# genetics-statistics/GEMMA

Hardware: AMD Instinct MI355X
Metric: SNPs/s (-lmm 1 Wald) at n=20k on 1/2/4/8 MI355X; U^T x HBM GB/s vs roofline (higher is better)
Workload: dtype f64 (U^T x as int8-digit MFMA products with exact int32 accumulation; every column of U scaled by its exact maximum and rounded to 6 base-256 digits = 2^-48 of that maximum -- fp64 keeps 2^-53 per entry; value_strict / strict_leg (7g6m: U^T x at or below the fp64 GEMM's own error) and fp64_gemm_path

## Files before the change

gemma_amd/_lib.py:

```python
import ctypes as C
import os

HERE = os.path.dirname(os.path.abspath(__file__))
LIB_PATH = os.path.join(HERE, "libgemma_hip.so")

SYMBOLS = [
    "gemma_hip_init", "gemma_hip_shutdown", "gemma_hip_abi_version", "gemma_hip_strerror",
    "gemma_hip_last_error", "gemma_hip_device_info", "gemma_hip_dgemm", "gemma_hip_dgemm_d",
    "gemma_hip_kin_begin", "gemma_hip_kin_add", "gemma_hip_kin_add_d", "gemma_hip_kin_end",
    "gemma_hip_kin_end_d", "gemma_hip_kin_loco_d", "gemma_hip_snp_qc", "gemma_hip_center", "gemma_hip_center_d", "gemma_hip_eigh",
    "gemma_hip_eigh_d", "gemma_hip_eigh_reserve", "gemma_hip_eigh_release", "gemma_hip_dbg_eigh_last", "gemma_hip_eigh_sharded_d", "gemma_hip_eigh_kept_K_sharded", "gemma_hip_calc_utx", "gemma_hip_lmm_setup", "gemma_hip_lmm_setup_d",
    "gemma_hip_lmm_null", "gemma_hip_lmm_set_indicator", "gemma_hip_lmm_batch", "gemma_hip_lmm_batch_d",
    "gemma_hip_lmm_assoc_d", "gemma_hip_lmm_finish", "gemma_hip_lm_setup", "gemma_hip_lm_batch", "gemma_hip_lm_batch_d",
    "gemma_hip_lm_finish", "gemma_hip_profile_enable",
    "gemma_hip_profile_read", "gemma_hip_dbg_tridiag", "gemma_hip_dbg_stedc", "gemma_hip_dbg_eigh2", "gemma_hip_dbg_utx", "gemma_hip_lmm_gene_batch", "gemma_hip_lmm_gene_batch_d", "gemma_hip_lmm_set_env",
    "gemma_hip_lmm_gxe_batch", "gemma_hip_lmm_gxe_batch_d",
    "gemma_hip_mvlmm_null", "gemma_hip_mvlmm_set", "gemma_hip_mvlmm_batch", "gemma_hip_mvlmm_batch_d",
    "gemma_hip_kin_end_keep", "gemma_hip_kept_K_get", "gemma_hip_eigh_kept_K", "gemma_hip_eigh_keep", "gemma_hip_kept_n",
    "gemma_hip_kept_bcast", "gemma_hip_kept_U_get", "gemma_hip_calc_utx_kept", "gemma_hip_lmm_setup_kept", "gemma_hip_kept_release",
    "gemma_hip_comm_unique_id", "gemma_hip_comm_init", "gemma_hip_comm_info", "gemma_hip_comm_bcast_d",
    "gemma_hip_comm_allreduce_sum_d", "gemma_hip_comm_finalize", "gemma_hip_comm_selftest", "gemma_hip_comm_stats", "gemma_hip_dbg_i8_digits", "gemma_hip_dbg_last_utx_path", "gemma_hip_lmm_batch_submit", "gemma_hip_lmm_batch_collect",
    "gemma_hip_dbg_last_utx_kernel", "gemma_hip_dbg_last_block_missing", "gemma_hip_dbg_last_i8_post", "gemma_hip_reload_env", "gemma_hip_lmm_batch_pipe_d", "gemma_hip_lmm_pipe_flush",
    "gemma_hip_spd_inverse", "gemma_hip_spd_inverse_d", "gemma_hip_vc_setup", "gemma_hip_vc_setup_d", "gemma_hip_vc_he",
    "gemma_hip_vc_reml", "gemma_hip_vc_timing", "gemma_hip_vc_release",
    "gemma_hip_ridge_setup", "gemma_hip_ridge_setup_d", "gemma_hip_ridge_setup_kept", "gemma_hip_ridge_set_r",
    "gemma_hip_ridge_set_indicator", "gemma_hip_ridge_batch", "gemma_hip_ridge_batch_d", "gemma_hip_ridge_finish",
    "gemma_hip_prdt_begin", "gemma_hip_prdt_add", "gemma_hip_prdt_add_d", "gemma_hip_prdt_add_bv", "gemma_hip_prdt_add_bv_d",
    "gemma_hip_prdt_end", "gemma_hip_prdt_kin", "gemma_hip_prdt_kin_mv_apply", "gemma_hip_prdt_kin_mv_apply_d", "gemma_hip_prdt_kin_mv",
    "gemma_hip_mqs_begin", "gemma_hip_mqs_add", "gemma_hip_mqs_add_d", "gemma_hip_mqs_end", "gemma_hip_mqs_get",
    "gemma_hip_mqs_S", "gemma_hip_mqs_S_d", "gemma_hip_mqs_release",
    "gemma_hip_cor_begin", "gemma_hip_cor_block", "gemma_hip_cor_block_d", "gemma_hip_cor_release",
    "gemma_hip_ci_begin", "gemma_hip_ci_xwz", "gemma_hip_ci_xwz_d", "gemma_hip_ci_xwz_end", "gemma_hip_ci_xtxwz",
    "gemma_hip_ci_xtxwz_d", "gemma_hip_ci_release",
    "gemma_hip_lmm_multi_setup", "gemma_hip_lmm_multi_setup_d", "gemma_hip_lmm_multi_setup_kept", "gemma_hip_lmm_multi_batch",
    "gemma_hip_lmm_multi_batch_d",
    "gemma_hip_lmm_score_panel_setup", "gemma_hip_lmm_score_panel_setup_d", "gemma_hip_lmm_score_panel_setup_kept",
    "gemma_hip_lmm_score_panel_batch", "gemma_hip_lmm_score_panel_batch_d", "gemma_hip_lmm_score_panel_assoc_d",
# ... 156 lines not shown
    L.gemma_hip_lmm_multi_batch_d.argtypes = [ci, vp, sz, sz, vp, vp]
    L.gemma_hip_lmm_score_panel_setup.argtypes = [C.POINTER(LmmCfg), sz, dp, dp, dp, dp, dp]
    L.gemma_hip_lmm_score_panel_setup_d.argtypes = [C.POINTER(LmmCfg), sz, dp, dp, dp, dp, dp, vp]
    L.gemma_hip_lmm_score_panel_setup_kept.argtypes = [C.POINTER(LmmCfg), sz, dp, dp, dp]
    L.gemma_hip_lmm_score_panel_batch.argtypes = [ci, vp, sz, sz, vp]
    L.gemma_hip_lmm_score_panel_batch_d.argtypes = [ci, vp, sz, sz, vp, vp]
    L.gemma_hip_lmm_score_panel_assoc_d.argtypes = [dp, sz, sz, vp, vp]
    L.gemma_hip_lmm_score_panel_hits_batch.argtypes = [ci, vp, sz, sz, C.c_double, vp, sz, vp, vp]
    L.gemma_hip_lmm_score_panel_hits_batch_d.argtypes = [ci, vp, sz, sz, C.c_double, vp, sz, vp, vp, vp]
    L.gemma_hip_lmm_score_panel_hits_assoc_d.argtypes = [dp, sz, sz, C.c_double, vp, sz, vp, vp, vp]
    L.gemma_hip_lmm_null_panel.argtypes = [sz, sz, sz, dp, dp, dp, cd, cd, sz, cd, vp, dp, dp]
    L.gemma_hip_lmm_null_panel_d.argtypes = [sz, sz, sz, dp, dp, dp, cd, cd, sz, cd, vp, dp, dp, vp]
    L.gemma_hip_dbg_i8_digits.argtypes = [sz, C.POINTER(ci)]
    L.gemma_hip_dbg_last_utx_path.argtypes = [C.POINTER(ci)]
    L.gemma_hip_dbg_last_utx_kernel.argtypes = [C.POINTER(UtxKernelInfo)]
    L.gemma_hip_dbg_last_block_missing.argtypes = [C.POINTER(ci)]
    L.gemma_hip_dbg_last_i8_post.argtypes = [C.POINTER(C.c_long), C.POINTER(C.c_long), C.POINTER(ci)]
    L.gemma_hip_reload_env.argtypes = []
    L.gemma_hip_lmm_batch_pipe_d.argtypes = [ci, vp, sz, sz, vp, vp]
    L.gemma_hip_lmm_pipe_flush.argtypes = [vp]
    L.gemma_hip_lmm_batch_submit.argtypes = [ci, vp, sz, sz]
    L.gemma_hip_lmm_batch_collect.argtypes = [vp, C.POINTER(sz)]
    L.gemma_hip_comm_unique_id.argtypes = [vp]
    L.gemma_hip_comm_init.argtypes = [vp, ci, ci]
    L.gemma_hip_comm_info.argtypes = [C.POINTER(ci), C.POINTER(ci), C.POINTER(ci)]
    L.gemma_hip_comm_bcast_d.argtypes = [vp, sz, ci, vp]
    L.gemma_hip_comm_allreduce_sum_d.argtypes = [dp, sz, vp]
    L.gemma_hip_comm_selftest.argtypes = [vp]
    L.gemma_hip_comm_stats.argtypes = [C.POINTER(CommStats)]
    L.gemma_hip_spd_inverse.argtypes = [dp, sz, sz, C.POINTER(cd), C.POINTER(C.c_long)]
# ... 56 lines not shown
```

gemma_amd/api.py:

```python
import collections
import ctypes as C

import numpy as np

from . import _lib as L

SUMSTAT_DTYPE = np.dtype([(k, "f8") for k in
                          ("beta", "se", "lambda_remle", "lambda_mle", "p_wald", "p_lrt", "p_score",
                           "logl_H1")])
SCORE_DTYPE = np.dtype([(k, "f8") for k in ("beta", "se", "p_score")])
SCORE_HIT_DTYPE = np.dtype([("snp", "u4"), ("pheno", "u4"), ("beta", "f8"), ("se", "f8"), ("p_score", "f8")])
SCORE_BEST_DTYPE = np.dtype([("beta", "f8"), ("se", "f8"), ("p_score", "f8"), ("snp", "i8")])
NULL_DTYPE = np.dtype([(k, "f8") for k in ("l_mle_null", "logl_mle_H0", "l_remle_null", "logl_remle_H0", "pve", "pve_se", "vg_remle",
                                             "ve_remle")])
LMM_BATCH_SIZE = 20000
K_BATCH_SIZE = 20000


def _is_torch(x):
    return type(x).__module__.startswith("torch")


def _np64(a, name):
    if not isinstance(a, np.ndarray) or a.dtype != np.float64:
# ... 77 lines not shown
    L.check(L.lib().gemma_hip_dbg_last_utx_path(C.byref(p)), "dbg_last_utx_path")
    return p.value


def last_utx_kernel():
    k = L.UtxKernelInfo()
    L.check(L.lib().gemma_hip_dbg_last_utx_kernel(C.byref(k)), "dbg_last_utx_kernel")
    return {"variant": k.variant, "rows": k.rows, "digits": k.digits, "fuse": k.fuse, "raster": k.raster,
            "launches": k.launches, "name": k.name.decode()}


def last_block_missing():
    a = C.c_int()
    L.check(L.lib().gemma_hip_dbg_last_block_missing(C.byref(a)), "dbg_last_block_missing")
    return a.value


def reload_env():
    L.check(L.lib().gemma_hip_reload_env(), "reload_env")


def fast_dgemm(TransA, TransB, alpha, A, B, beta, Cm):
    ta, tb = TransA.upper()[0], TransB.upper()[0]
    M, N = Cm.shape
    if ta not in "NT" or tb not in "NT":
        raise L.GemmaHipError(L.EINVAL, "fast_dgemm", "bad transpose flag")
    Ka = A.shape[0] if ta == "T" else A.shape[1]
    Ma = A.shape[1] if ta == "T" else A.shape[0]
    Kb = B.shape[1] if tb == "T" else B.shape[0]
    Nb = B.shape[0] if tb == "T" else B.shape[1]
# ... 1871 lines not shown
```

gemma_amd/csrc/abi_kept_comm.inc.h:

```cpp

extern "C" int gemma_hip_kin_end_keep(size_t *ns_used, int allreduce) {
  NEED_INIT();
  if (!g_ctx.kin_active) return fail(GEMMA_HIP_ESTATE, "kin_end before kin_begin");
  const size_t n = g_ctx.kin_n;
  size_t ns = g_ctx.kin_ns;
  {
    int rc = kin_fold_i8(nullptr);
    if (rc) return rc;
  }
  if (allreduce && g_ctx.comm.active && g_ctx.comm.world > 1) {
    std::string err;
    if (g_ctx.comm.allreduce_sum(g_ctx.kin_K.as<double>(), n * n, nullptr, err)) return fail(GEMMA_HIP_ERUNTIME, "%s", err.c_str());
    if (g_ctx.scratch.reserve(16)) return fail(GEMMA_HIP_ENOMEM, "kin_end_keep: scratch");
    double cnt = (double)ns;
    HIPCHK(hipMemcpy(g_ctx.scratch.p, &cnt, 8, hipMemcpyHostToDevice));
    if (g_ctx.comm.allreduce_sum(g_ctx.scratch.as<double>(), 1, nullptr, err)) return fail(GEMMA_HIP_ERUNTIME, "%s", err.c_str());
    HIPCHK(hipMemcpy(&cnt, g_ctx.scratch.p, 8, hipMemcpyDeviceToHost));
    ns = (size_t)(cnt + 0.5);
  }
  if (ns_used) *ns_used = ns;
  const double scale = ns ? 1.0 / (double)ns : 1.0;
  const unsigned nb = (unsigned)((n + 31) / 32);
  hipLaunchKernelGGL(symm_fill_scale_kernel, dim3(nb, nb), dim3(32, 8), 0, 0, g_ctx.kin_K.as<double>(), (long)n, (long)n,
                     scale);
// ... 309 lines not shown
  out->bcast_pieces = st.bcast_pieces;
  out->allreduce_bytes = st.allreduce_bytes;
  out->bcast_bytes = st.bcast_bytes;
  out->allreduce_s = st.allreduce_s;
  out->bcast_s = st.bcast_s;
  return GEMMA_HIP_OK;
}


extern "C" int gemma_hip_dbg_last_utx_kernel(gemma_utx_kernel_info *info) {
  if (!info) return fail(GEMMA_HIP_EINVAL, "dbg_last_utx_kernel: null");
  *info = g_ctx.last_utx_kernel;
  return GEMMA_HIP_OK;
}

extern "C" int gemma_hip_dbg_last_block_missing(int *any) {
  NEED_INIT();
  if (!any) return fail(GEMMA_HIP_EINVAL, "dbg_last_block_missing: null");
  *any = -1;
  if (g_ctx.i8_flag_at < 0 || !g_ctx.i8_rowsur.p) return GEMMA_HIP_OK;
  HIPCHK(hipDeviceSynchronize());
  HIPCHK(hipMemcpy(any, g_ctx.i8_rowsur.as<int>() + g_ctx.i8_flag_at, sizeof(int), hipMemcpyDeviceToHost));
  return GEMMA_HIP_OK;
}

extern "C" int gemma_hip_dbg_last_i8_post(long *short_rows, long *long_rows, int *epilogue) {
  NEED_INIT();
  if (!short_rows || !long_rows || !epilogue) return fail(GEMMA_HIP_EINVAL, "dbg_last_i8_post: null");
  *short_rows = *long_rows = -1;
  *epilogue = g_ctx.i8_last_epi;
// ... 30 lines not shown
```

gemma_amd/csrc/abi_lmm_stage.inc.h:

```cpp

static void slot_swap(Ctx::PhenoSlot &p) {
  std::swap(g_ctx.assoc_proto, p.proto);
  std::swap(g_ctx.Uty, p.Uty);
  std::swap(g_ctx.grid_R, p.grid_R); std::swap(g_ctx.grid_F, p.grid_F);
  std::swap(g_ctx.cheb_R, p.cheb_R); std::swap(g_ctx.cheb_F, p.cheb_F);
  std::swap(g_ctx.carry, p.carry);
  std::swap(g_ctx.carry_flip, p.carry_flip);
  std::swap(g_ctx.grid_geom, p.grid_geom); std::swap(g_ctx.cheb_geom, p.cheb_geom);
  std::swap(g_ctx.cheb_mid, p.cheb_mid); std::swap(g_ctx.cheb_inv_half, p.cheb_inv_half);
  std::swap(g_ctx.cheb_qmask, p.cheb_qmask);
}
static void multi_release() {
  for (auto &p : g_ctx.slots) {
    p.grid_R.release(); p.grid_F.release(); p.cheb_R.release(); p.cheb_F.release(); p.carry.release();
  }
  g_ctx.slots.clear();
  g_ctx.multi_Yt.release(); g_ctx.multi_R.release(); g_ctx.multi_T_buf.release();
  g_ctx.multi_T = 0;
  g_ctx.multi_G = 0;
}
static void score_release() {
  g_ctx.score_R.release(); g_ctx.score_Pyy.release(); g_ctx.score_Yt.release(); g_ctx.score_lam.release(); g_ctx.score_bad.release();
  g_ctx.score_fthr.release(); g_ctx.score_cells.release(); g_ctx.score_hits.release(); g_ctx.score_cnt.release(); g_ctx.score_best.release();
  g_ctx.score_fthr_p = -1.0;
// ... 228 lines not shown
  hipLaunchKernelGGL(grid_weights_kernel, dim3((unsigned)((r_elems + 255) / 256)), dim3(256), 0, s, k, gg, (int)c,
                     g_ctx.grid_R.as<double>());
  HIPCHK(hipGetLastError());
  hipLaunchKernelGGL(grid_fixed_kernel, dim3((unsigned)gg.nq), dim3(256), 0, s, k, (int)c, g_ctx.grid_F.as<double>());
  HIPCHK(hipGetLastError());
  g_ctx.grid_geom = gg;
  a.grid_F = g_ctx.grid_F.as<double>();
  a.grid_ld = (int)(nb * 16);
  a.grid_nq = gg.nq;
  a.grid_xa0 = gg.nbx * 16;
  a.have_grid = 1;
  return make_cheb(s);
}

static bool table_v2_enabled() { return g_ctx.knobs.table_v2 != 0; }
static int table_ksplit(int nc) { return std::max(1, std::min(16, nc / 32)); }
template <int NBX, int NBA, int RG>
static int launch_table_v2_t(const GridGeom &gg, const double *UtX, size_t l, size_t ld, const double *R, double *T,
                             const TableGather *tg, int nint, hipStream_t s) {
  constexpr int NB16 = (NBX + NBA) * 16;
  const size_t rows_per_block = (size_t)RG * 16 * 4;
  const size_t bx = (l + rows_per_block - 1) / rows_per_block;
  const int ksplit = table_ksplit(gg.nc);
  const size_t planes = tg ? (size_t)nint : 1;
  if (g_ctx.table_P.reserve(planes * (size_t)ksplit * l * NB16 * 8))
    return fail(GEMMA_HIP_ENOMEM, "lmm_assoc: table partial sums (%zu bytes)", planes * (size_t)ksplit * l * NB16 * 8);
  TableV2 a;
  a.UtX = UtX; a.ld = (long)ld; a.l = (long)l; a.n = (int)g_ctx.cfg.n; a.nc = gg.nc; a.ksplit = ksplit; a.Rp = R;
  a.P = g_ctx.table_P.as<double>(); a.cap = (long)l;
  if (tg) a.tg = *tg; else a.tg = TableGather();
  const long total = (long)l * NB16;
// ... 2 lines not shown
    if (pf) hipLaunchKernelGGL((table_v2_kernel<NBX, NBA, RG, true, true>), dim3((unsigned)bx, (unsigned)ksplit, (unsigned)nint), dim3(256), 0, s, a);
    else hipLaunchKernelGGL((table_v2_kernel<NBX, NBA, RG, true, false>), dim3((unsigned)bx, (unsigned)ksplit, (unsigned)nint), dim3(256), 0, s, a);
    HIPCHK(hipGetLastError());
    hipLaunchKernelGGL(table_reduce_kernel<true>, dim3((unsigned)((total + 255) / 256), (unsigned)nint), dim3(256), 0, s,
                       a.P, ksplit, a.cap, NB16, (long)l, tg->count, T);
  } else {
    if (pf) hipLaunchKernelGGL((table_v2_kernel<NBX, NBA, RG, false, true>), dim3((unsigned)bx, (unsigned)ksplit), dim3(256), 0, s, a);
    else hipLaunchKernelGGL((table_v2_kernel<NBX, NBA, RG, false, false>), dim3((unsigned)bx, (unsigned)ksplit), dim3(256), 0, s, a);
    HIPCHK(hipGetLastError());
    hipLaunchKernelGGL(table_reduce_kernel<false>, dim3((unsigned)((total + 255) / 256)), dim3(256), 0, s, a.P, ksplit,
                       a.cap, NB16, (long)l, (const int *)nullptr, T);
  }
  HIPCHK(hipGetLastError());
  return GEMMA_HIP_OK;
}
static int launch_table_v2(const GridGeom &gg, const double *UtX, size_t l, size_t ld, const double *R, double *T,
                           const TableGather *tg, int nint, hipStream_t s) {
  switch (gg.nba) {
  case 3: return launch_table_v2_t<2, 3, 4>(gg, UtX, l, ld, R, T, tg, nint, s);
  case 5: return launch_table_v2_t<2, 5, 2>(gg, UtX, l, ld, R, T, tg, nint, s);
  case 6: return launch_table_v2_t<2, 6, 2>(gg, UtX, l, ld, R, T, tg, nint, s);
  case 8: return launch_table_v2_t<2, 8, 2>(gg, UtX, l, ld, R, T, tg, nint, s);
  default: return fail(GEMMA_HIP_ERUNTIME, "lmm_assoc: no table kernel for %d column blocks", gg.nba);
  }
}

static int launch_grid_table(const double *UtX, size_t l, size_t ld, hipStream_t s) {
  const GridGeom &gg = g_ctx.grid_geom;
  const size_t nb = (size_t)(gg.nbx + gg.nba);
  if (g_ctx.grid_T.reserve(l * nb * 16 * 8)) return fail(GEMMA_HIP_ENOMEM, "lmm_assoc: fixed-lambda table");
  const unsigned grid = (unsigned)((l + 15) / 16);
  const double *R = g_ctx.grid_R.as<double>();
// ... 288 lines not shown
```

gemma_amd/csrc/gemma_hip.hip:

```cpp
#include <hip/hip_runtime.h>

#include <cmath>
#include <cstdarg>
#include <cstdio>
#include <cstdlib>
#include <cstring>
#include <string>
#include <vector>

#include "../../include/gemma_hip.h"
#include "tu_common.h"
#include "dgemm.h"
#include "eigh_tu.h"
#include "vc_tu.h"
#include "prdt_tu.h"
#include "mqs_tu.h"
#include "cor_tu.h"
#include "ingest.h"
#include "lm_assoc.h"
#include "lmm_assoc.h"
#include "lmm_grid.h"
#include "lmm_score_panel.h"
#include "lmm_null_panel.h"
#include "i8gemm.h"
#include "i8gemm_sparse.h"
#include "i8gemm_sparse2.h"
#include "i8gemm_sparse2_r16.h"
#include "plink_records.h"
#include "i8gemm_dense16.h"
#include "qc.h"
#include "mvlmm.hip.h"
#include "comm.hip.h"
#include "kin_i8.h"
#include "i8_plan.h"

using namespace gemma_hip;

namespace {

struct StageProf {
  std::vector<std::pair<hipEvent_t, hipEvent_t>> ev;
  double acc_ms = 0.0;
  long launches = 0;
};

struct Knobs {
  I8Switches i8;
  int i8_digits = 0;
  int i8_scale_max = 1;
  int dosage_i8 = 1;
  int dosage_rows = 16;
  int table_v2 = 1;
  int table_pf = 0;
  int multi_table = 1;
  int force_generic = 0;
  int assoc_variant = 44;
  int mvlmm_rt = 0;
  int pipe_cus = 64;
  int kin_i8 = 1, kin_upper = 1, kin_lists = 1, kin_lists_oom = 0;
  long long kin_list_cap = 0;
  static int geti(const char *name, int dflt) {
    const char *e = getenv(name);
    return (e && *e) ? atoi(e) : dflt;
  }
  void load() {
    i8.utx_i8 = geti("GEMMA_HIP_UTX_I8", 1);
    const int dg = geti("GEMMA_HIP_I8_DIGITS", 0);
    i8_digits = (dg == 6 || dg == 7) ? dg : 0;
// ... 14 lines not shown
    const char *eep = getenv("GEMMA_HIP_I8_EPILOGUE");
    i8.epilogue = (eep && eep[0] == '0') ? 0 : 1;
    i8.epi_depth = geti("GEMMA_HIP_I8_EPI_DEPTH", 4) <= 1 ? 1 : 4;
    const char *edr = getenv("GEMMA_HIP_I8_DIRECT");
    i8.direct = (edr && edr[0] == '0') ? 0 : 1;
    const char *ed = getenv("GEMMA_HIP_UTX_DOSAGE_I8");
    dosage_i8 = (ed && ed[0] == '0') ? 0 : 1;
    dosage_rows = geti("GEMMA_HIP_DOSAGE_ROWS", 16) == 32 ? 32 : 16;
    const char *eo = getenv("GEMMA_HIP_OVERLAP");
    i8.overlap = (eo && eo[0] == '1') ? 1 : 0;
    i8.chunks = geti("GEMMA_HIP_OVERLAP_CHUNKS", 4);
    const char *et = getenv("GEMMA_HIP_TABLE_V2");
    table_v2 = (et && et[0] == '0') ? 0 : 1;
    const char *ep = getenv("GEMMA_HIP_TABLE_PF");
    table_pf = (ep && ep[0] == '1') ? 1 : 0;
    const char *em = getenv("GEMMA_HIP_MULTI_TABLE");
    multi_table = (em && em[0] == '0') ? 0 : 1;
    const char *eg = getenv("GEMMA_HIP_FORCE_GENERIC");
    force_generic = (eg && eg[0] == '1') ? 1 : 0;
    assoc_variant = geti("GEMMA_HIP_ASSOC_VARIANT", 44);
    const char *er = getenv("GEMMA_HIP_MVLMM_RT");
    mvlmm_rt = (er && er[0] == '1') ? 1 : 0;
    pipe_cus = geti("GEMMA_HIP_PIPE_CUS", 64);
    const char *k1 = getenv("GEMMA_HIP_KIN_I8"), *k2 = getenv("GEMMA_HIP_KIN_UPPER"), *k3 = getenv("GEMMA_HIP_KIN_LISTS");
    const char *k4 = getenv("GEMMA_HIP_KIN_LISTS_OOM"), *k5 = getenv("GEMMA_HIP_KIN_LIST_CAP");
    kin_i8 = (k1 && k1[0] == '0') ? 0 : 1;
    kin_upper = (k2 && k2[0] == '0') ? 0 : 1;
    kin_lists = (k3 && k3[0] == '0') ? 0 : 1;
    kin_lists_oom = (k4 && k4[0] == '1') ? 1 : 0;
    kin_list_cap = (k5 && *k5) ? atoll(k5) : 0;
// ... 41 lines not shown
  } xp;
  int kin_tmap_tm = 0, kin_tmap_tn = 0, kin_tmap_count = 0;

  bool lmm_active = false;
  gemma_lmm_cfg cfg;
  const double *U = nullptr, *eval = nullptr, *Uty = nullptr;
  DevBuf own_U, own_eval, own_Uty, own_UtW, UtWt, idx_map;
  size_t ni_total = 0;
  bool have_map = false;
  DevBuf X, UtX, stage_in, stage_out, carry;
  DevBuf grid_R, grid_F, grid_T;
  DevBuf cheb_R, cheb_F, cheb_T, cheb_slots, cheb_list, cheb_count, cheb_D, cheb_Ck, cheb_Gk, cheb_Lk, cheb_iv, cheb_dends, cheb_res;
  double cheb_mid[ASSOC_MAX_REGION], cheb_inv_half[ASSOC_MAX_REGION];
  GridGeom cheb_geom;
  DevBuf table_P;
  DevBuf gxe_env, gxe_UtWt, gxe_Z, gxe_UtZ, gxe_flip;
  bool gxe_ready = false;
  double gxe_lnbeta = 0.0;
  DevBuf mv_Yt, mv_out;
  DevBuf mv_scratch;
  bool mv_ready = false, mv_gxe = false;
  size_t mv_d = 0;
  MvArgs mv_proto;
  DevBuf i8_Bt, i8_q, i8_qinv, i8_cmax, i8_A, i8_C, i8_mean;
  unsigned long long cheb_qmask = 0;
  struct RasterSlot {
    DevBuf dev;
    std::vector<int2> host;
    int tm = 0, tn = 0, rb = 0, xcds = 8;
    unsigned long long used = 0;
// ... 331 lines not shown
```

gemma_amd/csrc/lmm_grid.h:

```cpp
#pragma once
#include <hip/hip_runtime.h>
#include "dgemm.h"
#include "lmm_assoc.h"

namespace gemma_hip {

constexpr int GRID_FIX_LD = 16;

struct GridGeom {
  int nq;
  int nbx;
  int nba;
  int nc;
};

__global__ void grid_weights_kernel(AssocArgs g, GridGeom gg, int c, double *__restrict__ Rp);

__global__ __launch_bounds__(256) void grid_fixed_kernel(AssocArgs g, int c, double *__restrict__ F);

struct TableGather {
  const int *list;
  const int *count;
  long cap;
  long rp_stride;
// ... 2 lines not shown
template <int NBX, int NBA, bool GATHER>
__global__ __launch_bounds__(256) void grid_table_kernel(const double *__restrict__ UtX, long ld, long l, int n,
                                                        int nc, const double *__restrict__ Rp,
                                                        double *__restrict__ T, TableGather tg);

struct TableV2 {
  const double *UtX;
  long ld;
  long l;
  int n, nc;
  int ksplit;
  const double *Rp;
  double *P;
  long cap;
  TableGather tg;
};

template <int NBX, int NBA, int RG, bool GATHER, bool PF>
__global__ __launch_bounds__(256, PF ? 1 : 2) void table_v2_kernel(TableV2 a);

template <bool GATHER>
__global__ __launch_bounds__(256) void table_reduce_kernel(const double *__restrict__ P, int ksplit, long cap, int nb16,
                                                          long l, const int *__restrict__ count, double *__restrict__ T);

constexpr int MULTI_NBA = 8, MULTI_RG = 2, MULTI_GMAX = 4;
struct MultiWeights {
  const double *Uty[MULTI_GMAX];
  int G;
};

__global__ void grid_weights_multi_kernel(AssocArgs g, GridGeom gg, int c, MultiWeights mw, double *__restrict__ Rp);
struct TableMulti {
  const double *P;
  int ksplit;
// ... 61 lines not shown
  T void table_v2_kernel<2, 3, 4, false, true>(TableV2); \
  T void table_v2_kernel<2, 3, 4, true, false>(TableV2); \
  T void table_v2_kernel<2, 3, 4, true, true>(TableV2); \
  T void table_v2_kernel<2, 5, 2, false, false>(TableV2); \
  T void table_v2_kernel<2, 5, 2, false, true>(TableV2); \
  T void table_v2_kernel<2, 5, 2, true, false>(TableV2); \
  T void table_v2_kernel<2, 5, 2, true, true>(TableV2); \
  T void table_v2_kernel<2, 6, 2, false, false>(TableV2); \
  T void table_v2_kernel<2, 6, 2, false, true>(TableV2); \
  T void table_v2_kernel<2, 6, 2, true, false>(TableV2); \
  T void table_v2_kernel<2, 6, 2, true, true>(TableV2); \
  T void table_v2_kernel<2, 8, 2, false, false>(TableV2); \
  T void table_v2_kernel<2, 8, 2, false, true>(TableV2); \
  T void table_v2_kernel<2, 8, 2, true, false>(TableV2); \
  T void table_v2_kernel<2, 8, 2, true, true>(TableV2); \
  T void table_reduce_kernel<false>(const double *, int, long, int, long, const int *, double *); \
  T void table_reduce_kernel<true>(const double *, int, long, int, long, const int *, double *); \
  T void cheb_scan_kernel<1>(AssocArgs, ChebScanArgs); \
  T void cheb_scan_kernel<2>(AssocArgs, ChebScanArgs); \
  T void cheb_scan_kernel<3>(AssocArgs, ChebScanArgs); \
  T void cheb_scan_kernel<4>(AssocArgs, ChebScanArgs); \
  T void cheb_search_kernel<1>(AssocArgs, ChebSearchArgs); \
  T void cheb_search_kernel<2>(AssocArgs, ChebSearchArgs); \
  T void cheb_search_kernel<3>(AssocArgs, ChebSearchArgs); \
  T void cheb_search_kernel<4>(AssocArgs, ChebSearchArgs);
#ifndef GEMMA_HIP_KERNEL_BODIES
LMM_GRID_INSTANCES(extern template __global__)
#endif

}
// ... 1 lines not shown
```

gemma_amd/csrc/lmm_grid.hip.h:

```cpp
#pragma once
#include <hip/hip_runtime.h>
#include "dgemm.h"
#include "lmm_assoc.hip.h"
#define GEMMA_HIP_KERNEL_BODIES
#include "lmm_grid.h"

namespace gemma_hip {

__device__ __forceinline__ double grid_weight(const double *__restrict__ eval, const double *lam_grid, int q, long k) {
  if (q == 0) return 1.0;
  const int gi = (q - 1) >> 1;
  const double h = recip(eval[k] * lam_grid[gi] + 1.0);
  return ((q - 1) & 1) ? h * h : h;
}

__global__ void grid_weights_kernel(AssocArgs g, GridGeom gg, int c, double *__restrict__ Rp) {
  const long total = (long)gg.nc * (gg.nbx + gg.nba) * 256;
  const long e = (long)blockIdx.x * blockDim.x + threadIdx.x;
  if (e >= total) return;
  const int j = (int)(e & 3), col = (int)((e >> 2) & 15), kq = (int)((e >> 6) & 3);
  const long r = e >> 8;
  const int nb = gg.nbx + gg.nba;
  const int cb = (int)(r % nb);
  const long chunk = r / nb;
// ... 221 lines not shown
    TV2_MFMA(rbA, xvA);
  }
#undef TV2_LOAD
#undef TV2_MFMA
  double *P = a.P + ((long)(kint * a.ksplit + ks) * a.cap) * (NB * 16);
#pragma unroll
  for (int g = 0; g < RG; ++g)
#pragma unroll
    for (int b = 0; b < NB; ++b)
#pragma unroll
      for (int r = 0; r < 4; ++r) {
        const long srow = s0 + g * 16 + kq + 4 * r;
        if (srow < l) P[srow * (NB * 16) + b * 16 + i] = acc[g][b][r];
      }
}
template <bool GATHER>
__global__ __launch_bounds__(256) void table_reduce_kernel(const double *__restrict__ P, int ksplit, long cap, int nb16,
                                                          long l, const int *__restrict__ count, double *__restrict__ T) {
  const int kint = GATHER ? blockIdx.y : 0;
  if (GATHER) l = count[kint];
  const long e = (long)blockIdx.x * 256 + threadIdx.x;
  if (e >= l * nb16) return;
  const long row = e / nb16;
  const int col = (int)(e - row * nb16);
  const double *p = P + ((long)kint * ksplit * cap + row) * nb16 + col;
  double v = 0.0;
  for (int ks = 0; ks < ksplit; ++ks) v += p[(long)ks * cap * nb16];
  if (GATHER)
    T[((long)kint * nb16 + col) * cap + row] = v;
  else
// ... 231 lines not shown
```

include/gemma_hip.h:

```cpp
#ifndef GEMMA_HIP_H
#define GEMMA_HIP_H

#include <stddef.h>
#include <stdint.h>

#ifdef __cplusplus
extern "C" {
#endif

#define GEMMA_HIP_ABI_VERSION 4

enum {
  GEMMA_HIP_OK = 0,
  GEMMA_HIP_EINVAL = 1,
  GEMMA_HIP_ENODEV = 2,
  GEMMA_HIP_ENOMEM = 3,
  GEMMA_HIP_ERUNTIME = 4,
  GEMMA_HIP_ESTATE = 5,
  GEMMA_HIP_ENOCONV = 6,
  GEMMA_HIP_ENOTPD = 7
};

typedef struct {
  double beta, se, lambda_remle, lambda_mle, p_wald, p_lrt, p_score, logl_H1;
// ... 206 lines not shown
  GEMMA_UTX_KERNEL_RECORDS_R16 = 4,
  GEMMA_UTX_KERNEL_DOSAGE_I8 = 5,
  GEMMA_UTX_KERNEL_DOSAGE_I8_R16 = 6,
  GEMMA_UTX_KERNEL_COUNT = 7
};
typedef struct {
  int variant;
  int rows;
  int digits;
  int fuse;
  int raster;
  long launches;
  char name[64];
} gemma_utx_kernel_info;
int gemma_hip_dbg_last_utx_kernel(gemma_utx_kernel_info *info);
int gemma_hip_dbg_last_block_missing(int *any);
int gemma_hip_dbg_last_i8_post(long *short_rows, long *long_rows, int *epilogue);
int gemma_hip_reload_env(void);
int gemma_hip_dbg_i8_digits(size_t n, int *digits);

int gemma_hip_spd_inverse(double *A, size_t n, size_t lda, double *logdet, long *bad_pivot);
int gemma_hip_spd_inverse_d(double *A_d, size_t n, size_t lda, double *logdet, long *bad_pivot, void *stream);

int gemma_hip_vc_setup(size_t n, size_t n_vc, const double *const *K, size_t ldk, const double *W, size_t n_cvt, const double *y);
int gemma_hip_vc_setup_d(size_t n, size_t n_vc, const double *const *K_d, size_t ldk, const double *W, size_t n_cvt,
                         const double *y);
int gemma_hip_vc_he(double *sigma2, double *se_sigma2, double *pve, double *se_pve, double *pve_total, double *se_pve_total);
int gemma_hip_vc_reml(int noconstrain, double *sigma2, double *se_sigma2, double *pve, double *se_pve, double *pve_total,
                      double *se_pve_total, int *iterations, int *status, long *counts, double *iter_sigma2, size_t iter_cap);
int gemma_hip_vc_timing(double *t5);
// ... 61 lines not shown
```

Baseline: 364,700.

## Add double-buffered LDS table kernel with occupancy-aware row-group planning

Adds a table_v3 kernel that stages the R coefficients through double-buffered shared memory and prefetches the next chunk of R and UtX into registers while the current MFMA stage computes. A new planner picks the row-group count per workgroup so the last round of work items fills most CU slots, and caps the grid for the gathered case using a grid-stride loop. The default table form is set to 3, so dense (non-gather) table builds take the new path, while gather builds keep the old v2 kernel unless form 4 is requested. This adds LDS pressure and extra index arithmetic in exchange for hiding global-load latency and reducing tail imbalance.

```diff
diff --git a/gemma_amd/_lib.py b/gemma_amd/_lib.py
--- a/gemma_amd/_lib.py
+++ b/gemma_amd/_lib.py
@@ -20,7 +20,7 @@
     "gemma_hip_kept_bcast", "gemma_hip_kept_U_get", "gemma_hip_calc_utx_kept", "gemma_hip_lmm_setup_kept", "gemma_hip_kept_release",
     "gemma_hip_comm_unique_id", "gemma_hip_comm_init", "gemma_hip_comm_info", "gemma_hip_comm_bcast_d",
     "gemma_hip_comm_allreduce_sum_d", "gemma_hip_comm_finalize", "gemma_hip_comm_selftest", "gemma_hip_comm_stats", "gemma_hip_dbg_i8_digits", "gemma_hip_dbg_last_utx_path", "gemma_hip_lmm_batch_submit", "gemma_hip_lmm_batch_collect",
-    "gemma_hip_dbg_last_utx_kernel", "gemma_hip_dbg_last_block_missing", "gemma_hip_dbg_last_i8_post", "gemma_hip_reload_env", "gemma_hip_lmm_batch_pipe_d", "gemma_hip_lmm_pipe_flush",
+    "gemma_hip_dbg_last_utx_kernel", "gemma_hip_dbg_last_table", "gemma_hip_dbg_last_block_missing", "gemma_hip_dbg_last_i8_post", "gemma_hip_reload_env", "gemma_hip_lmm_batch_pipe_d", "gemma_hip_lmm_pipe_flush",
     "gemma_hip_spd_inverse", "gemma_hip_spd_inverse_d", "gemma_hip_vc_setup", "gemma_hip_vc_setup_d", "gemma_hip_vc_he",
     "gemma_hip_vc_reml", "gemma_hip_vc_timing", "gemma_hip_vc_release",
     "gemma_hip_ridge_setup", "gemma_hip_ridge_setup_d", "gemma_hip_ridge_setup_kept", "gemma_hip_ridge_set_r",
@@ -207,6 +207,7 @@
     L.gemma_hip_dbg_i8_digits.argtypes = [sz, C.POINTER(ci)]
     L.gemma_hip_dbg_last_utx_path.argtypes = [C.POINTER(ci)]
     L.gemma_hip_dbg_last_utx_kernel.argtypes = [C.POINTER(UtxKernelInfo)]
+    L.gemma_hip_dbg_last_table.argtypes = [C.POINTER(ci), C.POINTER(ci), C.POINTER(ci), C.POINTER(C.c_long)]
     L.gemma_hip_dbg_last_block_missing.argtypes = [C.POINTER(ci)]
     L.gemma_hip_dbg_last_i8_post.argtypes = [C.POINTER(C.c_long), C.POINTER(C.c_long), C.POINTER(ci)]
     L.gemma_hip_reload_env.argtypes = []
diff --git a/gemma_amd/api.py b/gemma_amd/api.py
--- a/gemma_amd/api.py
+++ b/gemma_amd/api.py
@@ -115,6 +115,12 @@
     a = C.c_int()
     L.check(L.lib().gemma_hip_dbg_last_block_missing(C.byref(a)), "dbg_last_block_missing")
     return a.value
+
+
+def last_table():
+    f, d, g, n = C.c_int(), C.c_int(), C.c_int(), C.c_long()
+    L.check(L.lib().gemma_hip_dbg_last_table(C.byref(f), C.byref(d), C.byref(g), C.byref(n)), "dbg_last_table")
+    return {"form": f.value, "rg_dense": d.value, "rg_gather": g.value, "launches": n.value}
 
 
 def reload_env():
diff --git a/gemma_amd/csrc/abi_kept_comm.inc.h b/gemma_amd/csrc/abi_kept_comm.inc.h
--- a/gemma_amd/csrc/abi_kept_comm.inc.h
+++ b/gemma_amd/csrc/abi_kept_comm.inc.h
@@ -347,6 +347,14 @@
   return GEMMA_HIP_OK;
 }
 
+extern "C" int gemma_hip_dbg_last_table(int *form, int *rg_dense, int *rg_gather, long *launches) {
+  if (launches) *launches = g_ctx.table_launches;
+  if (form) *form = g_ctx.last_table_form;
+  if (rg_dense) *rg_dense = g_ctx.last_table_rg[0];
+  if (rg_gather) *rg_gather = g_ctx.last_table_rg[1];
+  return GEMMA_HIP_OK;
+}
+
 extern "C" int gemma_hip_dbg_last_block_missing(int *any) {
   NEED_INIT();
   if (!any) return fail(GEMMA_HIP_EINVAL, "dbg_last_block_missing: null");
diff --git a/gemma_amd/csrc/abi_lmm_stage.inc.h b/gemma_amd/csrc/abi_lmm_stage.inc.h
--- a/gemma_amd/csrc/abi_lmm_stage.inc.h
+++ b/gemma_amd/csrc/abi_lmm_stage.inc.h
@@ -266,7 +266,6 @@
 }
 
 static bool table_v2_enabled() { return g_ctx.knobs.table_v2 != 0; }
-static int table_ksplit(int nc) { return std::max(1, std::min(16, nc / 32)); }
 template <int NBX, int NBA, int RG>
 static int launch_table_v2_t(const GridGeom &gg, const double *UtX, size_t l, size_t ld, const double *R, double *T,
                              const TableGather *tg, int nint, hipStream_t s) {
@@ -299,8 +298,65 @@
   HIPCHK(hipGetLastError());
   return GEMMA_HIP_OK;
 }
+template <int NBX, int NBA, int RG, bool GATHER>
+static void launch_table_v3_rg(const TablePlan &p, const TableV2 &a, hipStream_t s) {
+  hipLaunchKernelGGL((table_v3_kernel<NBX, NBA, RG, GATHER>), dim3(p.grid), dim3(256), 0, s, a);
+}
+template <int NBX, int NBA, bool GATHER>
+static int launch_table_v3_g(const TablePlan &p, const TableV2 &a, hipStream_t s) {
+  constexpr int NB = NBX + NBA;
+  switch (p.rg) {
+  case 1: launch_table_v3_rg<NBX, NBA, 1, GATHER>(p, a, s); break;
+  case 2:
+    if constexpr (NB <= 7) {
+      launch_table_v3_rg<NBX, NBA, 2, GATHER>(p, a, s);
+      break;
+    }
+  default: return fail(GEMMA_HIP_ERUNTIME, "lmm_assoc: no table kernel for %d row groups at %d column blocks", p.rg, NB);
+  }
+  return GEMMA_HIP_OK;
+}
+template <int NBX, int NBA>
+static int launch_table_v3_t(const GridGeom &gg, const double *UtX, size_t l, size_t ld, const double *R, double *T,
+                             const TableGather *tg, int nint, hipStream_t s) {
+  constexpr int NB16 = (NBX + NBA) * 16;
+  if (l == 0) return GEMMA_HIP_OK;
+  const TablePlan p = table_plan((long)l, gg.nc, g_ctx.prop.multiProcessorCount, NBX + NBA, tg ? nint : 0);
+  const size_t planes = tg ? (size_t)nint : 1;
+  if (g_ctx.table_P.reserve(planes * (size_t)p.ksplit * l * NB16 * 8))
+    return fail(GEMMA_HIP_ENOMEM, "lmm_assoc: table partial sums (%zu bytes)", planes * (size_t)p.ksplit * l * NB16 * 8);
+  TableV2 a;
+  a.UtX = UtX; a.ld = (long)ld; a.l = (long)l; a.n = (int)g_ctx.cfg.n; a.nc = gg.nc; a.ksplit = p.ksplit; a.Rp = R;
+  a.P = g_ctx.table_P.as<double>(); a.cap = (long)l; a.nint = tg ? nint : 0;
+  if (tg) a.tg = *tg; else a.tg = TableGather();
+  const long total = (long)l * NB16;
+  int rc = tg ? launch_table_v3_g<NBX, NBA, true>(p, a, s) : launch_table_v3_g<NBX, NBA, false>(p, a, s);
+  if (rc) return rc;
+  HIPCHK(hipGetLastError());
+  if (tg)
+    hipLaunchKernelGGL(table_reduce_kernel<true>, dim3((unsigned)((total + 255) / 256), (unsigned)nint), dim3(256), 0, s,
+                       a.P, p.ksplit, a.cap, NB16, (long)l, tg->count, T);
+  else
+    hipLaunchKernelGGL(table_reduce_kernel<false>, dim3((unsigned)((total + 255) / 256)), dim3(256), 0, s, a.P, p.ksplit,
+                       a.cap, NB16, (long)l, (const int *)nullptr, T);
+  HIPCHK(hipGetLastError());
+  g_ctx.last_table_form = g_ctx.knobs.table_form;
+  ++g_ctx.table_launches;
+  g_ctx.last_table_rg[tg ? 1 : 0] = p.rg;
+  return GEMMA_HIP_OK;
+}
 static int launch_table_v2(const GridGeom &gg, const double *UtX, size_t l, size_t ld, const double *R, double *T,
                            const TableGather *tg, int nint, hipStream_t s) {
+  if (g_ctx.knobs.table_form == 4 || (g_ctx.knobs.table_form == 3 && !tg)) switch (gg.nba) {
+  case 3: return launch_table_v3_t<2, 3>(gg, UtX, l, ld, R, T, tg, nint, s);
+  case 5: return launch_table_v3_t<2, 5>(gg, UtX, l, ld, R, T, tg, nint, s);
+  case 6: return launch_table_v3_t<2, 6>(gg, UtX, l, ld, R, T, tg, nint, s);
+  case 8: return launch_table_v3_t<2, 8>(gg, UtX, l, ld, R, T, tg, nint, s);
+  default: return fail(GEMMA_HIP_ERUNTIME, "lmm_assoc: no table kernel for %d column blocks", gg.nba);
+  }
+  g_ctx.last_table_form = g_ctx.knobs.table_form;
+  g_ctx.last_table_rg[tg ? 1 : 0] = 0;
+  ++g_ctx.table_launches;
   switch (gg.nba) {
   case 3: return launch_table_v2_t<2, 3, 4>(gg, UtX, l, ld, R, T, tg, nint, s);
   case 5: return launch_table_v2_t<2, 5, 2>(gg, UtX, l, ld, R, T, tg, nint, s);
diff --git a/gemma_amd/csrc/gemma_hip.hip b/gemma_amd/csrc/gemma_hip.hip
--- a/gemma_amd/csrc/gemma_hip.hip
+++ b/gemma_amd/csrc/gemma_hip.hip
@@ -33,6 +33,7 @@
 #include "comm.hip.h"
 #include "kin_i8.h"
 #include "i8_plan.h"
+#include "table_plan.h"
 
 using namespace gemma_hip;
 
@@ -52,6 +53,7 @@
   int dosage_rows = 16;
   int table_v2 = 1;
   int table_pf = 0;
+  int table_form = 3;
   int multi_table = 1;
   int force_generic = 0;
   int assoc_variant = 44;
@@ -96,6 +98,8 @@
     table_v2 = (et && et[0] == '0') ? 0 : 1;
     const char *ep = getenv("GEMMA_HIP_TABLE_PF");
     table_pf = (ep && ep[0] == '1') ? 1 : 0;
+    table_form = geti("GEMMA_HIP_TABLE_FORM", 3);
+    if (table_form != 2 && table_form != 4) table_form = 3;
     const char *em = getenv("GEMMA_HIP_MULTI_TABLE");
     multi_table = (em && em[0] == '0') ? 0 : 1;
     const char *eg = getenv("GEMMA_HIP_FORCE_GENERIC");
@@ -167,6 +171,8 @@
   double cheb_mid[ASSOC_MAX_REGION], cheb_inv_half[ASSOC_MAX_REGION];
   GridGeom cheb_geom;
   DevBuf table_P;
+  int last_table_form = 0, last_table_rg[2] = {0, 0};
+  long table_launches = 0;
   DevBuf gxe_env, gxe_UtWt, gxe_Z, gxe_UtZ, gxe_flip;
   bool gxe_ready = false;
   double gxe_lnbeta = 0.0;
diff --git a/gemma_amd/csrc/lmm_grid.h b/gemma_amd/csrc/lmm_grid.h
--- a/gemma_amd/csrc/lmm_grid.h
+++ b/gemma_amd/csrc/lmm_grid.h
@@ -40,10 +40,18 @@
   double *P;
   long cap;
   TableGather tg;
+  int nint;
 };
 
 template <int NBX, int NBA, int RG, bool GATHER, bool PF>
 __global__ __launch_bounds__(256, PF ? 1 : 2) void table_v2_kernel(TableV2 a);
+
+template <int NB>
+struct TableV3Stage {
+  static constexpr int SC = NB <= 5 ? 2 : 1;
+};
+template <int NBX, int NBA, int RG, bool GATHER>
+__global__ __launch_bounds__(256, 2) void table_v3_kernel(TableV2 a);
 
 template <bool GATHER>
 __global__ __launch_bounds__(256) void table_reduce_kernel(const double *__restrict__ P, int ksplit, long cap, int nb16,
@@ -135,6 +143,18 @@
   T void table_v2_kernel<2, 8, 2, false, true>(TableV2); \
   T void table_v2_kernel<2, 8, 2, true, false>(TableV2); \
   T void table_v2_kernel<2, 8, 2, true, true>(TableV2); \
+  T void table_v3_kernel<2, 3, 1, false>(TableV2); \
+  T void table_v3_kernel<2, 3, 1, true>(TableV2); \
+  T void table_v3_kernel<2, 3, 2, false>(TableV2); \
+  T void table_v3_kernel<2, 3, 2, true>(TableV2); \
+  T void table_v3_kernel<2, 5, 1, false>(TableV2); \
+  T void table_v3_kernel<2, 5, 1, true>(TableV2); \
+  T void table_v3_kernel<2, 5, 2, false>(TableV2); \
+  T void table_v3_kernel<2, 5, 2, true>(TableV2); \
+  T void table_v3_kernel<2, 6, 1, false>(TableV2); \
+  T void table_v3_kernel<2, 6, 1, true>(TableV2); \
+  T void table_v3_kernel<2, 8, 1, false>(TableV2); \
+  T void table_v3_kernel<2, 8, 1, true>(TableV2); \
   T void table_reduce_kernel<false>(const double *, int, long, int, long, const int *, double *); \
   T void table_reduce_kernel<true>(const double *, int, long, int, long, const int *, double *); \
   T void cheb_scan_kernel<1>(AssocArgs, ChebScanArgs); \
diff --git a/gemma_amd/csrc/lmm_grid.hip.h b/gemma_amd/csrc/lmm_grid.hip.h
--- a/gemma_amd/csrc/lmm_grid.hip.h
+++ b/gemma_amd/csrc/lmm_grid.hip.h
@@ -259,6 +259,173 @@
         if (srow < l) P[srow * (NB * 16) + b * 16 + i] = acc[g][b][r];
       }
 }
+template <int NBX, int NBA, int RG, bool GATHER>
+__global__ __launch_bounds__(256, 2) void table_v3_kernel(TableV2 a) {
+  constexpr int NB = NBX + NBA;
+  constexpr int SC = TableV3Stage<NB>::SC;
+  constexpr int PIECES = SC * NB * 128;
+  constexpr int NP = (PIECES + 255) / 256;
+  constexpr long ROWS = 4L * RG * 16;
+  __shared__ f64x2 rs[2][PIECES];
+  const int t = threadIdx.x;
+  const int lane = t & 63;
+  const int wave = __builtin_amdgcn_readfirstlane(t >> 6);
+  const int i = lane & 15, kq = lane >> 4;
+  const int n = a.n;
+  const int nfull = n / 16;
+  long nblk = (a.l + ROWS - 1) / ROWS;
+  if (GATHER) {
+    nblk = 0;
+    for (int k = 0; k < a.nint; ++k) nblk += (a.tg.count[k] + ROWS - 1) / ROWS;
+  }
+  const long nitems = nblk * a.ksplit;
+  for (long item = blockIdx.x; item < nitems; item += gridDim.x) {
+    const int ks = (int)(item / nblk);
+    long blk = item - (long)ks * nblk;
+    int kint = 0;
+    long l = a.l;
+    const double *Rp = a.Rp;
+    if (GATHER) {
+      for (;; ++kint) {
+        l = a.tg.count[kint];
+        const long nbk = (l + ROWS - 1) / ROWS;
+        if (blk < nbk) break;
+        blk -= nbk;
+      }
+      Rp += (long)kint * a.tg.rp_stride;
+    }
+    const long s0 = (blk * 4 + wave) * (RG * 16);
+    const bool active = s0 < l;
+    const double *xr[RG];
+#pragma unroll
+    for (int g = 0; g < RG; ++g) {
+      long row = s0 + g * 16 + i;
+      if (row >= l) row = l - 1;
+      if (GATHER) row = a.tg.list[(long)kint * a.tg.cap + row];
+      xr[g] = a.UtX + row * a.ld + 4 * kq;
+    }
+    const int c0 = (int)((long)a.nc * ks / a.ksplit), c1 = (int)((long)a.nc * (ks + 1) / a.ksplit);
+    const int cfull = c1 < nfull ? c1 : nfull;
+    const int nst = cfull > c0 ? (cfull - c0 + SC - 1) / SC : 0;
+    f64x4 acc[RG][NB];
+#pragma unroll
+    for (int g = 0; g < RG; ++g)
+#pragma unroll
+      for (int b = 0; b < NB; ++b) acc[g][b] = f64x4{0.0, 0.0, 0.0, 0.0};
+#define TV3_LOADR(SR, ST)                                                                                         \
+  do {                                                                                                            \
+    _Pragma("unroll") for (int p = 0; p < NP; ++p) {                                                              \
+      const int e = p * 256 + t;                                                                                  \
+      if (NP * 256 == PIECES || e < PIECES) {                                                                     \
+        int ch_ = c0 + (ST) * SC + e / (NB * 128);                                                                \
+        if (ch_ >= cfull) ch_ = cfull - 1;                                                                        \
+        SR[p] = *reinterpret_cast<const f64x2 *>(Rp + ((long)ch_ * (NB * 128) + e % (NB * 128)) * 2);             \
+      }                                                                                                           \
+    }                                                                                                             \
+  } while (0)
+#define TV3_STORER(SR, BUF)                                                                                       \
+  do {                                                                                                            \
+    _Pragma("unroll") for (int p = 0; p < NP; ++p) {                                                              \
+      const int e = p * 256 + t;                                                                                  \
+      if (NP * 256 == PIECES || e < PIECES) rs[BUF][e] = SR[p];                                                   \
+    }                                                                                                             \
+  } while (0)
+#define TV3_LOADX(XV, ST)                                                                                         \
+  do {                                                                                                            \
+    _Pragma("unroll") for (int q = 0; q < SC; ++q) {                                                              \
+      int ch_ = c0 + (ST) * SC + q;                                                                               \
+      if (ch_ >= cfull) ch_ = cfull - 1;                                                                          \
+      _Pragma("unroll") for (int g = 0; g < RG; ++g) {                                                            \
+        const f64x2 lo = *reinterpret_cast<const f64x2 *>(xr[g] + (long)ch_ * 16);                                \
+        const f64x2 hi = *reinterpret_cast<const f64x2 *>(xr[g] + (long)ch_ * 16 + 2);                            \
+        XV[q][g][0] = lo.x; XV[q][g][1] = lo.y; XV[q][g][2] = hi.x; XV[q][g][3] = hi.y;                           \
+      }                                                                                                           \
+    }                                                                                                             \
+  } while (0)
+#define TV3_MFMA(RB, XVQ)                                                                                         \
+  do {                                                                                                            \
+    _Pragma("unroll") for (int j = 0; j < 4; ++j) {                                                               \
+      _Pragma("unroll") for (int g = 0; g < RG; ++g) {                                                            \
+        const double xs = XVQ[g][j] * XVQ[g][j];                                                                  \
+        _Pragma("unroll") for (int b = 0; b < NB; ++b)                                                            \
+          acc[g][b] = __builtin_amdgcn_mfma_f64_16x16x4f64(b < NBX ? xs : XVQ[g][j], RB[b][j], acc[g][b], 0, 0, 0); \
+      }                                                                                                           \
+    }                                                                                                             \
+  } while (0)
+    f64x2 sr[NP];
+    double xv[SC][RG][4], xn[SC][RG][4];
+    if (nst > 0) {
+      TV3_LOADR(sr, 0);
+      TV3_LOADX(xv, 0);
+      TV3_STORER(sr, 0);
+    }
+    __syncthreads();
+    for (int st = 0; st < nst; ++st) {
+      const int cur = st & 1;
+      const int nx = st + 1 < nst ? st + 1 : st;
+      TV3_LOADR(sr, nx);
+      TV3_LOADX(xn, nx);
+      __builtin_amdgcn_sched_barrier(0);
+      if (active) {
+#pragma unroll
+        for (int q = 0; q < SC; ++q) {
+          if (c0 + st * SC + q < cfull) {
+            double rb[NB][4];
+#pragma unroll
+            for (int b = 0; b < NB; ++b) {
+              const f64x2 lo = rs[cur][((q * NB + b) * 64 + lane) * 2];
+              const f64x2 hi = rs[cur][((q * NB + b) * 64 + lane) * 2 + 1];
+              rb[b][0] = lo.x; rb[b][1] = lo.y; rb[b][2] = hi.x; rb[b][3] = hi.y;
+            }
+            TV3_MFMA(rb, xv[q]);
+          }
+        }
+      }
+      __builtin_amdgcn_sched_barrier(0);
+      TV3_STORER(sr, cur ^ 1);
+      __syncthreads();
+#pragma unroll
+      for (int q = 0; q < SC; ++q)
+#pragma unroll
+        for (int g = 0; g < RG; ++g)
+#pragma unroll
+          for (int j = 0; j < 4; ++j) xv[q][g][j] = xn[q][g][j];
+    }
+    if (active && c1 > nfull && c0 <= nfull) {
+      const int ch = nfull;
+      const long k = (long)ch * 16 + 4 * kq;
+      const double *rp_ = Rp + (long)lane * 4 + (long)ch * NB * 256;
+      double rb[NB][4];
+#pragma unroll
+      for (int b = 0; b < NB; ++b) {
+        const f64x2 lo = *reinterpret_cast<const f64x2 *>(rp_ + (long)b * 256);
+        const f64x2 hi = *reinterpret_cast<const f64x2 *>(rp_ + (long)b * 256 + 2);
+        rb[b][0] = lo.x; rb[b][1] = lo.y; rb[b][2] = hi.x; rb[b][3] = hi.y;
+      }
+#pragma unroll
+      for (int g = 0; g < RG; ++g)
+#pragma unroll
+        for (int j = 0; j < 4; ++j) xv[0][g][j] = (k + j < n) ? xr[g][(long)ch * 16 + j] : 0.0;
+      TV3_MFMA(rb, xv[0]);
+    }
+#undef TV3_LOADR
+#undef TV3_STORER
+#undef TV3_LOADX
+#undef TV3_MFMA
+    double *P = a.P + ((long)(kint * a.ksplit + ks) * a.cap) * (NB * 16);
+    if (active) {
+#pragma unroll
+      for (int g = 0; g < RG; ++g)
+#pragma unroll
+        for (int b = 0; b < NB; ++b)
+#pragma unroll
+          for (int r = 0; r < 4; ++r) {
+            const long srow = s0 + g * 16 + kq + 4 * r;
+            if (srow < l) P[srow * (NB * 16) + b * 16 + i] = acc[g][b][r];
+          }
+    }
+  }
+}
 template <bool GATHER>
 __global__ __launch_bounds__(256) void table_reduce_kernel(const double *__restrict__ P, int ksplit, long cap, int nb16,
                                                           long l, const int *__restrict__ count, double *__restrict__ T) {
diff --git a/gemma_amd/csrc/table_plan.h b/gemma_amd/csrc/table_plan.h
--- /dev/null
+++ b/gemma_amd/csrc/table_plan.h
@@ -0,0 +1,78 @@
+#pragma once
+
+namespace gemma_hip {
+
+inline int table_ksplit(int nc) {
+  const int k = nc / 32;
+  return k < 1 ? 1 : k > 16 ? 16 : k;
+}
+
+constexpr int TABLE_WG_PER_CU = 2;
+constexpr int TABLE_WAVES = 4;
+constexpr double TABLE_MIN_LAST_ROUND = 0.75;
+
+inline int table_rg_max(int nb) { return nb <= 7 ? 2 : 1; }
+
+struct TablePlan {
+  int ksplit;
+  int rg;
+  long rows_per_wg;
+  long row_blocks;
+  long items;
+  long slots;
+  unsigned grid;
+  double last_round;
+  bool meets;
+};
+constexpr int TABLE_GATHER_ROUNDS = 8;
+
+inline long table_items(long l, int rg, int ksplit) {
+  const long rows = (long)TABLE_WAVES * rg * 16;
+  return (l + rows - 1) / rows * ksplit;
+}
+inline double table_last_round(long items, long slots) {
+  const long rem = items % slots;
+  return (items == 0 || rem == 0) ? 1.0 : (double)rem / (double)slots;
+}
+
+inline TablePlan table_plan(long l, int nc, int cus, int nb, int nint) {
+  TablePlan p;
+  p.ksplit = table_ksplit(nc);
+  p.slots = (long)(cus < 1 ? 1 : cus) * TABLE_WG_PER_CU;
+  const int rgmax = table_rg_max(nb);
+  int rg = 0;
+  for (int r = rgmax; r >= 1 && !rg; --r) {
+    const long it = table_items(l, r, p.ksplit);
+    if (it > p.slots ? table_last_round(it, p.slots) >= TABLE_MIN_LAST_ROUND : r == 1) rg = r;
+  }
+  if (!rg) {
+    long best = -1;
+    for (int r = rgmax; r >= 1; --r) {
+      const long it = table_items(l, r, p.ksplit);
+      const long cost = (it + p.slots - 1) / p.slots * r;
+      if (best < 0 || cost < best) { best = cost; rg = r; }
+    }
+  }
+  p.rg = rg;
+  p.rows_per_wg = (long)TABLE_WAVES * rg * 16;
+  p.row_blocks = (l + p.rows_per_wg - 1) / p.rows_per_wg;
+  const long dense_items = p.row_blocks * p.ksplit;
+  p.last_round = table_last_round(dense_items, p.slots);
+  p.meets = dense_items <= p.slots || p.last_round >= TABLE_MIN_LAST_ROUND;
+  if (nint > 0) {
+    p.items = dense_items * nint;
+    const long cap = (long)TABLE_GATHER_ROUNDS * p.slots;
+    p.grid = (unsigned)(p.items < cap ? p.items : cap);
+  } else {
+    p.items = dense_items;
+    p.grid = (unsigned)dense_items;
+  }
+  return p;
+}
+
+inline void table_item(const TablePlan &p, long item, long &row_block, int &ks) {
+  ks = (int)(item / p.row_blocks);
+  row_block = item - (long)ks * p.row_blocks;
+}
+
+}
diff --git a/include/gemma_hip.h b/include/gemma_hip.h
--- a/include/gemma_hip.h
+++ b/include/gemma_hip.h
@@ -244,6 +244,7 @@
   char name[64];
 } gemma_utx_kernel_info;
 int gemma_hip_dbg_last_utx_kernel(gemma_utx_kernel_info *info);
+int gemma_hip_dbg_last_table(int *form, int *rg_dense, int *rg_gather, long *launches);
 int gemma_hip_dbg_last_block_missing(int *any);
 int gemma_hip_dbg_last_i8_post(long *short_rows, long *long_rows, int *epilogue);
 int gemma_hip_reload_env(void);
```

Result: no change. 365,400, median of 2 (+0.2%).
